# Jarvis73/PEMP

Measured on AMD Instinct MI355X. Metric: episodes/sec (PEMP stage-1 eval step, PASCAL-5i-shaped 1-shot, ResNet-50), higher is better.
Workload: dtype f32

## Files before the change

### pemp_amd/build.py

```python
import hashlib
import os
import subprocess
from concurrent.futures import ThreadPoolExecutor

HERE = os.path.dirname(os.path.abspath(__file__))
CSRC = os.path.join(HERE, "csrc")
OBJ = os.path.join(HERE, "_obj")
OUT = os.path.join(HERE, "libpemp_hip.so")
SOURCES = ("conv_igemm.hip", "conv_dma.hip", "conv_dma2.hip", "conv_panel.hip", "conv_row3.hip", "conv_stem_pool.hip", "conv_wgrad.hip", "train_ops.hip", "pool_misc.hip", "head.hip", "head_bwd.hip", "cedt.hip",
           "episode_io.hip", "dropout.hip", "cm_linear.hip", "pfenet.hip", "pfenet_bwd.hip", "canet.hip", "canet_bwd.hip", "rpmms.hip", "rpmms_bwd.hip")
FLAGS = ["-O3", "--offload-arch=gfx950", "-std=c++17", "-fPIC"]


def _headers():
    return [os.path.join(CSRC, f) for f in sorted(os.listdir(CSRC)) if f.endswith((".h", ".inc"))] + \
           [os.path.join(HERE, "..", "include", "pemp_hip.h")]


def csrc_digest():
    h = hashlib.sha1()
    for f in sorted(os.listdir(CSRC)):
        with open(os.path.join(CSRC, f), "rb") as fh:
            h.update(f.encode() + b"\0" + fh.read())
    with open(os.path.join(HERE, "..", "include", "pemp_hip.h"), "rb") as fh:
        h.update(fh.read())
    return h.hexdigest()[:12]


CONV_ENGINE = ("common.h", "conv_common.h", "conv_tiles.h", "conv_igemm.hip", "conv_dma.hip", "conv_dma2.hip", "conv_panel.hip", "conv_row3.hip", "conv_stem_pool.hip")


def conv_digest():
    h = hashlib.sha1()
    for f in CONV_ENGINE:
        with open(os.path.join(CSRC, f), "rb") as fh:
            h.update(f.encode() + b"\0" + fh.read())
    return h.hexdigest()[:12]


def needs_build():
    if not os.path.exists(OUT):
        return True
    t = os.path.getmtime(OUT)
    deps = [os.path.join(CSRC, f) for f in os.listdir(CSRC)] + [os.path.join(HERE, "..", "include", "pemp_hip.h")]
    return any(os.path.getmtime(d) > t for d in deps)


def _stamp(src, flags):
    h = hashlib.sha1(" ".join(flags).encode())
    for f in [src] + _headers():
        with open(f, "rb") as fh:
            h.update(fh.read())
# ... 41 lines not shown
```

### pemp_amd/csrc/conv_common.h

```cpp
#pragma once
#include "common.h"

namespace pemp {

typedef __attribute__((ext_vector_type(16))) float f32x16;
typedef __attribute__((ext_vector_type(4))) float v4f;
typedef __attribute__((ext_vector_type(8))) __bf16 bf16x8;
typedef __attribute__((ext_vector_type(2))) unsigned int u32x2;

#define PEMP_CONV_BF16_IO 0x100u

__device__ __forceinline__ v4f load_quad(const float* base, size_t off, unsigned bf16) {
    if (!bf16) return *(const v4f*)(base + off);
    const u32x2 r = *(const u32x2*)((const unsigned short*)base + off);
    return v4f{__builtin_bit_cast(float, r.x << 16), __builtin_bit_cast(float, r.x & 0xFFFF0000u),
               __builtin_bit_cast(float, r.y << 16), __builtin_bit_cast(float, r.y & 0xFFFF0000u)};
}

__device__ __forceinline__ unsigned int bf16_bits(float f) {
    const unsigned int u = __builtin_bit_cast(unsigned int, f);
    if ((u & 0x7FFFFFFFu) > 0x7F800000u) return (u >> 16) | 0x40u;
    return (u + 0x7FFFu + ((u >> 16) & 1u)) >> 16;
}

// ... 349 lines not shown

int launch_conv_dma(int shape, const ConvArgs& a, hipStream_t st);
bool conv_dma2_supported(const ConvArgs& a);
int launch_conv_dma2(int shape, const ConvArgs& a, hipStream_t st);
int launch_conv_dma2_group(int shape, ConvGroupArgs& g, hipStream_t st);
int launch_conv_dma2_hybrid(const ConvArgs& a, hipStream_t st);
int conv_dma2_hybrid_rows(int M, int Cout);
int launch_conv_dma2_bf16(int shape, const ConvArgs& a, hipStream_t st);
int launch_conv_dma2_db(int shape, ConvArgs a, void* ws, size_t ws_bytes, bool split, hipStream_t st);
struct SplitKPlan { int full, split, pieces; size_t ws_bytes; };
SplitKPlan conv_dma2_splitk_plan(int shape, const ConvArgs& a);
int launch_conv_dma2_splitk(int shape, ConvArgs a, void* ws, size_t ws_bytes, hipStream_t st);
int launch_conv_dma2_split3(int shape, ConvArgs a, void* ws, size_t ws_bytes, bool split, hipStream_t st);
int launch_conv_dma2_group_split3(int shape, ConvGroupArgs& g, hipStream_t st);
int launch_conv_dma2_split3_stats(int shape, const ConvArgs& a, hipStream_t st);
bool conv_dma2_split3_stats_shape(int shape);
int launch_conv_dma2_split3_persist(int shape, const ConvArgs& a, hipStream_t st);
bool conv_dma2_persist_out_split3(int shape);
int launch_conv_dma2_split3_pre(int shape, bool persistent, const ConvArgs& a, hipStream_t st);
bool conv_panel_supported(const ConvArgs& a);
int launch_conv_panel(int shape, const ConvArgs& a, hipStream_t st);
bool conv_row3_supported(const ConvArgs& a);
int launch_conv_row3(bool persistent, const ConvArgs& a, hipStream_t st);
int conv_dma2_simds();
int pack_split3(const float* w, void* out, int cout, int kpad, hipStream_t st);
int launch_conv_stem_pool(const ConvArgs& a, hipStream_t st);
int conv_stem_pool_out(int i);

template <class Kern> int allow_lds(Kern kern, size_t lds);
template <class Kern>
int persistent_grid(Kern kern, int threads, size_t lds, long long tiles, int& occ_cache, const char* what, int& grid_out) {
    if (!occ_cache) {
        const int rc = allow_lds(kern, lds);
        if (rc) return rc;
        int v = 0;
        hipError_t e = hipOccupancyMaxActiveBlocksPerMultiprocessor(&v, (const void*)kern, threads, lds);
        if (e != hipSuccess || v <= 0) {
            set_error("%s: occupancy query failed (%s, %d blocks)", what, hipGetErrorString(e), v);
            return -1;
        }
        occ_cache = v;
    }
    long long grid = (long long)occ_cache * (conv_dma2_simds() / 4);
    if (grid < 8) grid = 8;
    if (grid > tiles) grid = tiles;
    grid_out = (int)grid;
// ... 5 lines not shown
```

### pemp_amd/csrc/conv_igemm.hip

```cpp
#include "conv_tiles.h"

namespace pemp {


template <int BM, int BN, int WGM, bool STEM>
__global__ __launch_bounds__(256) void conv_igemm_kernel(ConvArgs a) {
    constexpr int WGN = 4 / WGM;
    constexpr int WM = BM / WGM, WN = BN / WGN;
    constexpr int TM = WM / 32, TN = WN / 32;
    constexpr int AL = BM / 32, BL = BN / 32;
    static_assert(TM >= 1 && TN >= 1, "wave tile");

    extern __shared__ __attribute__((aligned(16))) v4f smem[];
    v4f* As = smem;
    v4f* Bs = smem + 2 * 8 * BM;

    const int tid = threadIdx.x;
    const int lane = tid & 63;
    const int wave = tid >> 6;
    const int wm0 = (wave / WGN) * WM;
    const int wn0 = (wave % WGN) * WN;
    const int lr = lane & 31, lh = lane >> 5;

    const int ntn = a.Cout / BN;
// ... 255 lines not shown
    a.dil = d->dil; a.ldr = d->ldr; a.Kpad = d->Kpad; a.flags = d->flags;
    a.HoWo = d->Ho * d->Wo;
    a.M = d->N * a.HoWo;
    a.ntaps = ntaps;
    a.cin_steps = stem ? 1 : d->Cin / 32;
    a.nk = d->Kpad / 32;
    if (residual && !(d->flags & PEMP_CONV_OUT_SPLIT3_ALSO)) PEMP_REQUIRE(d->ldr >= d->Cout && d->ldr % 4 == 0 && ((uintptr_t)residual & 15) == 0, "conv2d: ldr must be >= Cout and x4, residual 16-byte aligned");
    a.sk_ws = nullptr; a.sk_cnt = nullptr; a.sk_full = 0; a.sk_S = 1;
    a.bm_first = 0;
    return 0;
}

static int conv2d_impl(const pemp_conv_desc* d, const float* x, const float* w, float* y, const float* scale, const float* shift,
                       const float* residual, const float* pad_value, void* ws, size_t ws_bytes, void* stream) {
    ConvArgs a;
    const int rc = conv_fill(d, x, w, y, scale, shift, residual, pad_value, a, false, true);
    if (rc) return rc;
    const bool stem = d->flags & PEMP_CONV_STEM4;
    int tile = d->tile;
    if (tile == 0) {
        tile = 3;
    }
    TileId t = decode_tile(tile);
    const bool out_split3 = d->flags & PEMP_CONV_OUT_SPLIT3;
    if (out_split3)
        PEMP_REQUIRE(t.family == TILE_SPLIT3 && !t.splitk && !t.panel && !ws && !stem && !residual && a.Cout % 32 == 0 && a.ldy == a.Cout,
                     "conv2d: PEMP_CONV_OUT_SPLIT3 needs an unsplit split3 tile id (41..44, 46, 47, 49, 146, 149), ldy == Cout, no residual / workspace");
    const bool also_split3 = d->flags & PEMP_CONV_OUT_SPLIT3_ALSO;
    if (also_split3) {
        PEMP_REQUIRE(t.presplit && !out_split3 && !ws && !stem && a.Cout % 32 == 0,
                     "conv2d: PEMP_CONV_OUT_SPLIT3_ALSO needs tile id 146 / 149, no PEMP_CONV_OUT_SPLIT3 / split-K / workspace / stem");
        PEMP_REQUIRE(residual && ((uintptr_t)residual & 15) == 0,
                     "conv2d: PEMP_CONV_OUT_SPLIT3_ALSO takes the pre-split tensor (16-byte aligned) in the residual argument; a residual is never read");
        const char *y0 = (const char*)y, *y1 = y0 + ((size_t)(a.M - 1) * a.ldy + a.Cout) * 4;
        const char *s0 = (const char*)residual, *s1 = s0 + (size_t)a.M * a.Cout * 6;
        PEMP_REQUIRE(y1 <= s0 || s1 <= y0, "conv2d: PEMP_CONV_OUT_SPLIT3_ALSO: y and the pre-split tensor overlap");
    }
    const bool res_s2 = d->flags & PEMP_CONV_RES_S2;
    PEMP_REQUIRE(res_s2 || !(d->flags & (PEMP_CONV_RES_HEVEN | PEMP_CONV_RES_WEVEN)), "conv2d: PEMP_CONV_RES_HEVEN / _WEVEN come with PEMP_CONV_RES_S2");
    if (res_s2) {
        PEMP_REQUIRE(residual && !out_split3 && !also_split3 && !(d->flags & PEMP_CONV_IN_SPLIT3) && !ws && !stem && !pad_value,
                     "conv2d: PEMP_CONV_RES_S2 needs a residual, no pre-split operands / PEMP_CONV_OUT_SPLIT3_ALSO / split-K / workspace / stem / padding value");
        PEMP_REQUIRE(t.family == TILE_SPLIT3 && t.exists && !t.splitk && !t.persistent && !t.presplit &&
                         (t.panel ? (a.nk == 2 || (a.nk == 4 && t.shape == 2)) : t.shape == 3),
                     "conv2d: PEMP_CONV_RES_S2 needs tile id 43, 72 with Kpad 64 or 128, or 71 with Kpad 64 (tile %d, Kpad %d: the persistent, split-K, "
                     "pre-split and fp32-chain ids have no strided-residual form)", tile, a.Kpad);
// ... 294 lines not shown
```

### pemp_amd/csrc/conv_tiles.h

```cpp
#pragma once
#include <initializer_list>
#include "conv_common.h"

namespace pemp {

struct TileShape { int bm, bn, wgm, nw, wgm3; };
inline constexpr TileShape kTileShapes[10] = {
    {0, 0, 0, 0, 0},
    {128, 128, 2, 4, 4},
    {128, 64, 2, 4, 4},
    {64, 64, 2, 4, 2},
    {128, 128, 4, 8, 4},
    {128, 64, 4, 8, 0},
    {256, 128, 4, 8, 8},
    {256, 256, 4, 8, 0},
    {32, 64, 2, 4, 0},
    {64, 64, 2, 4, 0},
};

template <int S, bool S3 = false>
struct Tile {
    static constexpr int BM = kTileShapes[S].bm, BN = kTileShapes[S].bn, NW = kTileShapes[S].nw;
    static constexpr int WGM = S3 ? kTileShapes[S].wgm3 : kTileShapes[S].wgm;
};
// ... 17 lines not shown
template <class Fam, int S = 1, class F>
int with_tile(int shape, F&& f) {
    if constexpr (S > 9) {
        set_error("conv: tile shape %d outside the kernel family", shape);
        return -1;
    } else {
        if constexpr ((Fam::shapes >> S) & 1u) {
            if (shape == S) return f(Tile<S, Fam::s3>{});
        }
        return with_tile<Fam, S + 1>(shape, f);
    }
}

enum TileFamily { TILE_NONE = 0, TILE_IGEMM, TILE_DMA, TILE_DMA2, TILE_SPLIT3 };
struct TileId {
    int family;
    int shape;
    bool splitk;
    bool persistent;
    bool exists;
    bool panel;
    bool presplit;
    bool row3;
};

inline TileId decode_tile(int id) {
    TileId t = {TILE_NONE, 0, false, false, false, false, false, false};
    const int decade = id / 10, s = id % 10;
    if (id == 146 || id == 149 || id == 246 || id == 249) {
        t.family = TILE_SPLIT3, t.shape = 6, t.exists = t.presplit = true, t.persistent = id % 10 == 9, t.row3 = id > 200;
        return t;
    }
    if (decade == 7 && in_family<FamPanel>(s)) {
        t.family = TILE_SPLIT3, t.shape = s, t.exists = t.panel = true;
        return t;
    }
    if (id < 1 || id > 56 || s == 0) return t;
    t.shape = s;
    if (decade == 0) t.family = TILE_IGEMM, t.exists = in_family<FamIgemm>(s);
    else if (decade == 1) t.family = TILE_DMA, t.exists = in_family<FamFp32>(s);
    else if (decade == 2) t.family = TILE_DMA2, t.exists = true;
    else if (decade == 3) t.family = TILE_DMA2, t.splitk = true, t.exists = in_family<FamSplitK>(s);
    else if (decade == 4 && (s == 7 || s == 9)) t.family = TILE_SPLIT3, t.persistent = t.exists = true, t.shape = s == 7 ? 3 : 6;
    else if (decade == 4) t.family = TILE_SPLIT3, t.exists = in_family<FamSplit3>(s);
    else t.family = TILE_SPLIT3, t.splitk = true, t.exists = in_family<FamSplit3>(s) && in_family<FamSplitK>(s);
    return t;
}

inline bool tile_cout_ok(int shape, int Cout) { return Cout % kTileShapes[shape].bn == 0; }
#define PEMP_REQUIRE_COUT(who, shape, Cout)                                                                              \
    do {                                                                                                                 \
// ... 39 lines not shown
```

### pemp_amd/ops.py

```python
import ctypes as C
import collections
import functools
import json
import os

import torch

from . import _lib
from ._lib import ConvDesc, CONV_RELU, CONV_SHIFT_PER_IMAGE, CONV_STEM4, CONV_POOL3S2, CONV_OUT_SPLIT3, CONV_IN_SPLIT3, CONV_OUT_SPLIT3_ALSO
from ._lib import CONV_RES_S2, CONV_RES_HEVEN, CONV_RES_WEVEN


def _stream():
    return C.c_void_p(torch.cuda.current_stream().cuda_stream)


def _p(t):
    return C.c_void_p(t.data_ptr()) if t is not None else C.c_void_p(0)


def _chk_dev(*ts):
    for t in ts:
        if t is not None and (not t.is_cuda):
            raise _lib.PempHipError("pemp_amd ops need device (cuda/HIP) tensors; there is no CPU path")
# ... 26 lines not shown
    def __init__(self, w, scale, shift, cin, cout, kh, kw, stride, pad, dil, kpad, stem, relu, w3=None, w3pool=None):
        self.w, self.scale, self.shift, self.w3, self.w3pool = w, scale, shift, w3, w3pool
        self.cin, self.cout, self.kh, self.kw = cin, cout, kh, kw
        self.stride, self.pad, self.dil, self.kpad, self.stem, self.relu = stride, pad, dil, kpad, stem, relu


_SHAPES = {1: (128, 128), 2: (128, 64), 3: (64, 64), 4: (128, 128), 5: (128, 64), 6: (256, 128), 7: (256, 256),
           8: (32, 64),
           9: (64, 64)}
Tile = collections.namedtuple("Tile", "shape family splitk persistent_of")
SPLIT3_PERSISTENT = {47: 43, 49: 46}
TILES = {base + s: Tile(_SHAPES[s], family, base in (30, 50), None)
         for family, base, shapes in (("igemm", 0, (1, 2, 3)),
                                      ("dma", 10, range(1, 8)),
                                      ("dma2", 20, range(1, 10)),
                                      ("dma2", 30, (1, 2, 4, 5, 6, 7)),
                                      ("split3", 40, (1, 2, 3, 4, 6)),
                                      ("split3", 50, (1, 2, 4, 6)))
         for s in shapes}
TILES.update({t: TILES[of]._replace(persistent_of=of) for t, of in SPLIT3_PERSISTENT.items()})
TILES.update({70 + s: Tile(_SHAPES[s], "split3", False, None) for s in (1, 2)})
TILES.update({146: Tile(_SHAPES[6], "split3", False, None), 149: Tile(_SHAPES[6], "split3", False, 146)})
TILES.update({246: Tile(_SHAPES[6], "split3", False, None), 249: Tile(_SHAPES[6], "split3", False, 246)})
_NO_TILE = Tile(None, None, False, None)


def tile_shape(t):
    return TILES.get(t, _NO_TILE).shape


TILE_VARIANTS = {t: TILES[t].shape for t in (13, 14, 12, 11, 15, 3, 17, 16, 23, 24, 22, 21, 25, 27, 26, 28, 29)}
SPLIT3_TILES = (43, 42, 41, 44, 46, 47, 49)
SPLIT3_SPLITK_TILES = (51, 52, 54, 56)
SPLIT3_DEFAULT_TILE = 43
SPLIT3_PANEL_TILES = (71, 72)
SPLIT3_PANEL = os.environ.get("PEMP_SPLIT3_PANEL", "1") != "0"
SPLIT3_PRESPLIT_TILES = (146, 149)
SPLIT3_PRESPLIT = os.environ.get("PEMP_SPLIT3_PRESPLIT", "1") != "0"
SPLIT3_ROW3_TILES = (246, 249)
SPLIT3_ROW3 = os.environ.get("PEMP_SPLIT3_ROW3", "1") != "0"
ROW3_STAGE_ROWS = 288
AUTOTUNE = True
PICK_HOOK = None
SPLITK = os.environ.get("PEMP_CONV_SPLITK", "1") != "0"
DEFAULT_TILE = 13
_TILE_CACHE = {}
_TILE_CACHE_FILE = os.environ.get("PEMP_TILE_CACHE")
WGRAD_PICKS = {}
if _TILE_CACHE_FILE and os.path.exists(_TILE_CACHE_FILE):
    with open(_TILE_CACHE_FILE) as _f:
        for _k, _v in json.load(_f).items():
            _key = json.loads(_k)
            if _key and _key[0] == "wgrad":
                WGRAD_PICKS[tuple(_key[1:])] = tuple(_v) if isinstance(_v, list) else int(_v)
            else:
                _TILE_CACHE[tuple(_key)] = int(_v)


def save_picks():
    if not _TILE_CACHE_FILE:
        return
    out = {json.dumps([int(v) for v in k]): t for k, t in _TILE_CACHE.items()}
    out.update({json.dumps(["wgrad"] + [int(v) for v in k]): (list(t) if isinstance(t, tuple) else t) for k, t in WGRAD_PICKS.items()})
    with open(_TILE_CACHE_FILE, "w") as f:
# ... 100 lines not shown
            and pad_value is None and not splitk and not per_image_shift and n * h * w * ldx * 4 < lim
            and n * ho * wo * max(ldy, ldr) * 4 < lim)


SPLIT3_RES_S2_TILES = (43, 72, 71)


def res_s2_tiles(p):
    if p.w3 is None or p.stem:
        return ()
    panel = p.kh == 1 and p.kw == 1 and p.pad == 0
    return tuple(t for t in SPLIT3_RES_S2_TILES
                 if t == 43 or (panel and p.cout % _tile_bn(t) == 0 and (p.kpad == 64 or (p.kpad == 128 and t == 72))))


def row3_stage_rows(w, dil):
    return 256 + 2 * dil + dil * ((255 + 2 * dil + w - 1) // w)


def _row3_ok(p, w, residual, pad_value, out_split3, also_split3, per_image_shift):
    return (SPLIT3_ROW3 and (p.kh, p.kw, p.stride) == (3, 3, 1) and p.pad == p.dil and residual is None
            and pad_value is None and not out_split3 and also_split3 is None and not per_image_shift
            and row3_stage_rows(w, p.dil) <= ROW3_STAGE_ROWS)


def pack_split3(w):
    co, kpad = w.shape
    if w.dtype != torch.float32 or not w.is_contiguous() or kpad % 32:
        raise ValueError("pack_split3: a contiguous fp32 [Cout, Kpad] with Kpad % 32 == 0")
    out = torch.empty((co, kpad // 32, 3, 32), dtype=torch.bfloat16, device=w.device)
    _lib.check(_lib.load().pemp_pack_split3_bf16(_p(w), _p(out), co, kpad, _stream()), "pemp_pack_split3_bf16")
    return out


def hybrid_rows(n, ho, wo, cout):
    d = ConvDesc(n, ho, wo, 32, 32, ho, wo, cout, cout, 1, 1, 1, 0, 1, 0, 32, 0, 29)
    return int(_lib.load().pemp_conv2d_hybrid_rows(C.byref(d)))


def pack_conv_weight(w_oihw, stem4=False):
    co, ci, kh, kw = w_oihw.shape
    w = w_oihw.detach().permute(0, 2, 3, 1).contiguous().float()
    if stem4:
        if ci > 4:
            raise ValueError("stem4 packing needs Cin <= 4")
        k = kh * kw * 4
# ... 44 lines not shown
        raise ValueError(f"{who}: out shape {tuple(out.shape)} != {(n, ho, wo, p.cout)}")
    ldr = 0
    if residual is not None:
        ldr = _nhwc(residual, "residual", dtype)
        if residual_stride == 2:
            rn, hr, wr, rc = residual.shape
            if (rn, rc) != (n, p.cout) or (hr - 1) // 2 + 1 != ho or (wr - 1) // 2 + 1 != wo:
                raise ValueError(f"{who}: a stride-2 residual of shape {tuple(residual.shape)} does not cover the output {tuple(out.shape)}")
        elif tuple(residual.shape) != tuple(out.shape):
            raise ValueError(f"{who}: residual shape mismatch")
    elif residual_stride != 1:
        raise ValueError(f"{who}: residual_stride without a residual")
    return n, h, w, cin, ldx, ho, wo, out, ldy, ldr


def conv2d(x, p, out=None, residual=None, shift_override=None, per_image_shift=False, relu=None, tile=0,
           pad_value=None, splitk=False, dropblock=None, out_split3=False, x_split3=False, also_split3=None, residual_stride=1):
    if out_split3 or x_split3:
        what = "a pre-split output" if out_split3 else "a pre-split input"
        if p.w3 is None or p.stem:
            raise ValueError(f"conv2d: {what} needs a split3 layer (ConvParams.w3), not the fp32 chain or a stem")
        if splitk or dropblock is not None:
            raise ValueError(f"conv2d: {what} has no split-K / DropBlock form")
        if out_split3 and tile and (tile not in SPLIT3_TILES + SPLIT3_PRESPLIT_TILES):
            raise ValueError(f"conv2d: a pre-split output needs an unsplit split3 tile id, got {tile}")
        if x_split3 and (p.kh * p.kw == 1 or per_image_shift or p.cin % 32 or p.cout % 128):
            raise ValueError("conv2d: a pre-split input needs a multi-tap conv with Cin % 32 == 0 and Cout % 128 == 0, no per-image shift")
    if also_split3 is not None and (not x_split3 or out_split3 or residual is not None):
        raise ValueError("conv2d: a second, pre-split output needs a pre-split input (x_split3), no out_split3, no residual")
    if (tile in SPLIT3_PRESPLIT_TILES + SPLIT3_ROW3_TILES) != bool(x_split3) and (tile or not x_split3):
        raise ValueError(f"conv2d: the tile ids {SPLIT3_PRESPLIT_TILES + SPLIT3_ROW3_TILES} and x_split3 come together (tile {tile})")
    res_s2 = residual_stride == 2
    if residual_stride not in (1, 2):
        raise ValueError(f"conv2d: residual_stride must be 1 or 2, got {residual_stride}")
    if res_s2:
        if p.w3 is None or p.stem or x.dtype != torch.float32:
            raise ValueError("conv2d: a stride-2 residual needs a split3 layer (ConvParams.w3) on fp32 activations")
        if residual is None or out_split3 or x_split3 or also_split3 is not None or pad_value is not None or splitk or dropblock is not None:
            raise ValueError("conv2d: a stride-2 residual comes with a residual and without pre-split operands, padding value, split-K or DropBlock")
        if tile and tile not in res_s2_tiles(p):
            raise ValueError(f"conv2d: a stride-2 residual needs one of the tile ids {res_s2_tiles(p)} for this layer, got {tile}")
    if x.dtype == torch.bfloat16 and not x_split3:
        return _conv2d_bf16(x, p, out, residual, shift_override, per_image_shift, relu, tile, pad_value)
    n, h, w, cin, ldx, ho, wo, out, ldy, ldr = _conv_geom("conv2d", x, p, out, residual, x_split3=x_split3, out_split3=out_split3,
                                                          residual_stride=residual_stride)
    if also_split3 is not None and _split3_dims(also_split3, "also_split3") != (n, ho, wo, p.cout):
        raise ValueError(f"conv2d: also_split3 shape {tuple(also_split3.shape)} != {split3_shape(n, ho, wo, p.cout)}")
# ... 54 lines not shown
            ws, ws_bytes = _splitk_ws(lib, d, x.device)
            _check_sk(lib, lib.pemp_conv2d_padv_splitk_nhwc_f32(C.byref(d), _p(x), _p(pw), _p(out), _p(p.scale), _p(shift), _p(residual),
                                                                _p(pad_value), C.c_void_p(ws), ws_bytes, _stream()), ws,
                      "pemp_conv2d_padv_splitk_nhwc_f32")
        elif sk:
            ws, ws_bytes = _splitk_ws(lib, d, x.device)
            _check_sk(lib, lib.pemp_conv2d_splitk_nhwc_f32(C.byref(d), _p(x), _p(pw), _p(out), _p(p.scale), _p(shift), _p(residual),
                                                           C.c_void_p(ws), ws_bytes, _stream()), ws, "pemp_conv2d_splitk_nhwc_f32")
        elif pad_value is None:
            _lib.check(lib.pemp_conv2d_nhwc_f32(C.byref(d), _p(x), _p(pw), _p(out), _p(p.scale), _p(shift),
                                                _p(residual), _stream()), "pemp_conv2d_nhwc_f32")
        else:
            _lib.check(lib.pemp_conv2d_padv_nhwc_f32(C.byref(d), _p(x), _p(pw), _p(out), _p(p.scale), _p(shift),
                                                     _p(residual), _p(pad_value), _stream()), "pemp_conv2d_padv_nhwc_f32")

    if tile == 0:
        key = (p.cin, p.cout, p.kh, p.kw, p.stride, p.pad, p.dil, (6 if dropblock is not None else 4) if splitk else int(p.stem) + (7 if dropblock is not None else 0),
               n, h, w, int(residual is not None and also_split3 is None), int(pad_value is not None)) + ((3,) if s3 else ())
        if x_split3 or out_split3:
            key += (146,) * int(x_split3) + (17,) * int(out_split3) + (64,) * int(also_split3 is not None)
            row3 = bool(x_split3) and _row3_ok(p, w, residual, pad_value, out_split3, also_split3, per_image_shift)
            if row3:
                key += (246,)
            cands = lambda: _fits(list(SPLIT3_PRESPLIT_TILES if x_split3 else SPLIT3_TILES) +
                                  (list(SPLIT3_ROW3_TILES) if row3 and PICK_HOOK is None else []), p.cout)
        elif res_s2:
            panel = _panel_ok(p, n, ho, wo, ldx, ldy, ldr, h, w, pad_value, splitk, per_image_shift) \
                and residual.numel() // p.cout * ldr * 4 < 1 << 31
            key += (128,) + ((71,) if panel else ())
            cands = lambda: _fits([t for t in res_s2_tiles(p) if panel or t not in SPLIT3_PANEL_TILES], p.cout)
        elif s3:
            panel = _panel_ok(p, n, ho, wo, ldx, ldy, ldr, h, w, pad_value, splitk, per_image_shift)
            if panel:
                key += (71,)
            cands = lambda: _fits(list(SPLIT3_TILES) + (list(SPLIT3_SPLITK_TILES) if splitk else []) +
                                  (list(SPLIT3_PANEL_TILES) if panel else []), p.cout)
        else:
            def cands():
                ids = list(GROUP_TILES if dropblock is not None else TILE_VARIANTS) + (list(SPLITK_TILES) if splitk else [])
                if 29 in ids and not (hybrid_rows(n, ho, wo, p.cout) and dma2_supported(x, p)):
                    ids.remove(29)
                return _fits(ids, p.cout)
        tile = _choose_tile(key, n * ho * wo, launch, cands,
                            SPLIT3_PRESPLIT_TILES[0] if x_split3 else SPLIT3_DEFAULT_TILE if s3 else DEFAULT_TILE + (10 if dropblock is not None else 0))
    launch(tile)
    return out


def stem_pool_supported(p):
    return (p.stem and p.w3pool is not None and (p.kh, p.kw, p.stride, p.pad, p.dil) == (7, 7, 2, 3, 1) and p.kpad == 224
            and p.cout % 64 == 0)


def stem_pool(x, p, out=None):
    lib = _lib.load()
    if not stem_pool_supported(p):
        raise ValueError("stem_pool: a 7x7 / stride 2 / pad 3 NHWC4 stem with split weights (ConvParams.w3pool)")
    _chk_dev(x, p.w3pool, out)
    ldx = _nhwc(x, "x")
# ... 1091 lines not shown
```

### scratch/conv_trace_layers.py

```python
import collections
import csv
import sys

trace, per_step = sys.argv[1], int(sys.argv[2])
steps = int(sys.argv[3]) if len(sys.argv) > 3 else 20
rows = sorted(csv.DictReader(open(trace)), key=lambda r: int(r["Start_Timestamp"]))
conv = [r for r in rows if any(k in r["Kernel_Name"] for k in ("conv_dma", "conv_igemm", "conv_stem_pool", "conv_panel", "conv_row3"))][-steps * per_step:]
dur = lambda r: (int(r["End_Timestamp"]) - int(r["Start_Timestamp"])) / 1e3
pos = collections.defaultdict(list)
for i, r in enumerate(conv):
    pos[i % per_step].append(r)
print(f"conv launches per step {per_step}, steps {steps}: conv {sum(map(dur, conv)) / steps / 1e3:.3f} ms per step")
print(f"{'pos':>3} {'mean us':>9} {'grid':>8} {'wg':>4}  kernel")
for p in range(per_step):
    rs = pos[p]
    r = rs[-1]
    name = r["Kernel_Name"].split("(")[0].replace("void pemp::", "").replace("pemp::", "")
    g = r.get("Grid_Size", r.get("Grid_Size_X", "")); wg = r.get("Workgroup_Size", r.get("Workgroup_Size_X", ""))
    print(f"{p:>3} {sum(map(dur, rs)) / len(rs):9.1f} {g:>8} {wg:>4}  {name}")
```

### scratch/s3_layers_bench.py

```python
import argparse
import hashlib
import os
import sys

import torch

sys.path.insert(0, os.path.dirname(os.path.dirname(os.path.abspath(__file__))))
from pemp_amd import ops

UNSPLIT = (43, 42, 41, 44, 46, 47, 49)
SPLIT = (52, 51, 54, 56)
PANEL = ops.SPLIT3_PANEL_TILES
PRESPLIT = ops.SPLIT3_PRESPLIT_TILES
ROW3 = ops.SPLIT3_ROW3_TILES
LAYERS = ((256, 1024, 1, 1, True, False), (512, 1024, 1, 1, False, False), (1024, 256, 1, 1, False, False),
          (256, 256, 3, 2, False, False), (128, 512, 1, 1, True, False), (1024, 512, 1, 1, False, False),
          (256, 256, 3, 2, False, True),
          (64, 256, 1, 1, True, False, 1, 101), (64, 256, 1, 1, False, False, 1, 101), (256, 512, 1, 1, False, False, 2, 101),
          (128, 128, 3, 1, False, False), (128, 128, 3, 1, False, False, 2, 101), (64, 64, 3, 1, False, False, 1, 101),
          (512, 128, 1, 1, False, False),
          (64, 256, 1, 1, True, False, 1, 51, 101),
          (64, 64, 3, 1, False, False, 2, 101),
          (256, 256, 3, 12, False, True))


def timed(fn, reps, n=5):
    for _ in range(2):
        fn()
    e0, e1 = torch.cuda.Event(enable_timing=True), torch.cuda.Event(enable_timing=True)
    best, worst = 1e9, 0.0
    for _ in range(reps):
        e0.record()
        for _ in range(n):
            fn()
        e1.record()
        e1.synchronize()
        us = e0.elapsed_time(e1) / n * 1e3
        best, worst = min(best, us), max(worst, us)
    return best, worst


def presplit(x):
    h = x.to(torch.bfloat16)
# ... 15 lines not shown
    packed = packed.contiguous()
    prm = ops.ConvParams(packed, None, torch.randn(cout, generator=g).to(dev), cin, cout, 1, 1, 1, 0, 1, kpad, False, True, ops.pack_split3(packed))
    res = torch.randn(N, HR, HR, cout, generator=g).to(dev)
    ref = ops.conv2d(x, prm, residual=res[:, ::2, ::2, :].contiguous(), tile=43).clone()
    out = torch.empty_like(ref)
    fl = 2.0 * N * HW * HW * cout * cin
    cells = []
    for tile in keep(ops.res_s2_tiles(prm)):
        run = lambda: ops.conv2d(x, prm, residual=res, residual_stride=2, out=out, tile=tile)
        out.zero_()
        run()
        same = torch.equal(out, ref)
        us, worst = timed(run, reps)
        cells.append(f"{tile}: {us:7.1f}..{worst:6.1f}us {fl / us / 1e6:5.1f}TF{'' if same else ' !'}")
    print(f"{name:>16} k1 d1 res1 | " + " | ".join(cells), flush=True)
    print(f"{'':>16} hash 43={digest(ref)}", flush=True)


def main():
    ap = argparse.ArgumentParser()
    ap.add_argument("--only", default="", help="cin-cout-kK[-padv]: one layer")
    ap.add_argument("--reps", type=int, default=3)
    ap.add_argument("--ids", default="", help="comma-separated tile ids: only these are timed (a counter run of one kernel)")
    ap.add_argument("--res", type=int, choices=(0, 1), default=None, help="run the selected layers without / with a residual, whatever their row says")
    args = ap.parse_args()
    dev = torch.device("cuda:0")
    N = 50
    keep = lambda ids: tuple(t for t in ids if not args.ids or str(t) in args.ids.split(","))
    for layer in LAYERS:
        cin, cout, k, dil, has_res, padv = layer[:6]
        stride, HW = layer[6:8] if len(layer) > 6 else (1, 51)
        RS2 = layer[8] if len(layer) > 8 else 0
        has_res = has_res if args.res is None or RS2 else bool(args.res)
        M = N * HW * HW
        HO = (HW - 1) // stride + 1
        name = f"{cin}-{cout}-k{k}" + (f"-d{dil}" if k == 3 and dil > 2 else "") + ("-padv" if padv else "") + (f"-s{stride}" if stride > 1 else "") + (f"-hw{HW}-res{int(has_res)}" if HW != 51 else "") + ("-rs2" if RS2 else "")
        if args.only and name not in args.only.split(","):
            continue
        if RS2:
            rs2_row(dev, N, HW, RS2, cin, cout, name, keep, args.reps)
            continue
        g = torch.Generator().manual_seed(cin * 7 + cout * 3 + k)
        buf = torch.empty(M + 4, cin, device=dev)
        buf[:M] = torch.randn(M, cin, generator=g).to(dev)
        buf[M:] = torch.randn(cin, generator=g).to(dev)
        x, pv = buf[:M].view(N, HW, HW, cin), buf[M]
        w = (torch.randn(cout, cin, k, k, generator=g) * (1.0 / (cin * k * k) ** 0.5)).to(dev)
        packed, kpad = ops.pack_conv_weight(w)
        packed = packed.contiguous()
        prm = ops.ConvParams(packed, None, torch.randn(cout, generator=g).to(dev), cin, cout, k, k, stride, dil if k == 3 else 0, dil, kpad,
                             False, True, ops.pack_split3(packed))
        res = torch.randn(N, HO, HO, cout, generator=g).to(dev) if has_res else None
        pad_value = pv if padv else None
        out = torch.empty(N, HO, HO, cout, device=dev)
        fl = 2.0 * N * HO * HO * cout * k * k * cin
        ref = ops.conv2d(x, prm, residual=res, pad_value=pad_value, tile=43).clone()
        cells, hashes = [], [f"43={digest(ref)}"]
        panel = PANEL if k == 1 and kpad <= 256 and not padv else ()
        for tile in keep(UNSPLIT + panel + SPLIT):
            if cout % ops._tile_bn(tile):
                continue
            run = lambda: ops.conv2d(x, prm, residual=res, pad_value=pad_value, out=out, tile=tile)
            run()
            same = torch.equal(out, ref)
            if tile in SPLIT:
                hashes.append(f"{tile}=" + ("43" if same else digest(out)))
            us, worst = timed(run, args.reps)
            mark = "" if same else (" ~" if tile in SPLIT else " !")
            cells.append(f"{tile}: {us:7.1f}..{worst:6.1f}us {fl / us / 1e6:5.1f}TF{mark}")
            if tile not in SPLIT and not same:
                hashes.append(f"{tile}=MISMATCH:{digest(out)}")
        if k > 1 and cout % 128 == 0:
            sbuf = torch.zeros((M + 4) * cin * 3, dtype=torch.bfloat16, device=dev)
            sbuf[:(M + 1) * cin * 3] = presplit(buf[:M + 1]).reshape(-1)
            xs, pvs = sbuf[:M * cin * 3].view(N, HW, HW, cin // 32, 3, 32), sbuf[M * cin * 3:(M + 1) * cin * 3].view(cin // 32, 3, 32)
            row3 = ROW3 if k == 3 and stride == 1 and not has_res and not padv and ops.row3_stage_rows(HW, dil) <= ops.ROW3_STAGE_ROWS else ()
            for tile in keep(PRESPLIT + row3):
                run = lambda: ops.conv2d(xs, prm, residual=res, pad_value=pvs if padv else None, out=out, tile=tile, x_split3=True)
                out.zero_()
                run()
                same = torch.equal(out, ref)
                us, worst = timed(run, args.reps)
                cells.append(f"{tile}: {us:7.1f}..{worst:6.1f}us {fl / us / 1e6:5.1f}TF{'' if same else ' !'}")
            if not has_res:
                want = presplit(ref)
                outs = torch.empty_like(want)
                for tile in keep(PRESPLIT):
                    run = lambda: ops.conv2d(xs, prm, pad_value=pvs if padv else None, out=out, tile=tile, x_split3=True, also_split3=outs)
                    out.zero_()
                    run()
                    same = torch.equal(out, ref) and torch.equal(outs.view(torch.int16), want.view(torch.int16))
                    us, worst = timed(run, args.reps)
                    cells.append(f"{tile}+s: {us:7.1f}..{worst:6.1f}us{'' if same else ' !'}")
                del want, outs
            del sbuf, xs, pvs
        if k == 1 and not has_res:
            want = presplit(ref)
            outs = torch.empty_like(want)
            for tile in keep((43, 42, 41, 44, 46, 47, 49) if not args.ids else ()):
                if cout % ops._tile_bn(tile):
                    continue
                run = lambda: ops.conv2d(x, prm, out=outs, tile=tile, out_split3=True)
                run()
                same = torch.equal(outs.view(torch.int16), want.view(torch.int16))
                us, worst = timed(run, args.reps)
                cells.append(f"{tile}s: {us:7.1f}..{worst:6.1f}us{'' if same else ' !'}")
            del want, outs
        print(f"{name:>16} k{k} d{dil} res{int(has_res)} | " + " | ".join(cells), flush=True)
        print(f"{'':>16} hash " + " ".join(hashes), flush=True)
    print("(146 / 149 / 246 / 249: on the pre-split input; NNs: id NN writing a pre-split output, ! = not the split of id 43's;")
    print(" NNN+s: id NNN writing fp32 and the pre-split copy, ! = either differs)")
    print("(! = an unsplit id differs from id 43; ~ = a split-K id differs from id 43, expected where it splits)")


if __name__ == "__main__":
    main()
```

Measured before the change: 1552.

## Add persistent triple-buffered ring conv kernel for 1x1 split3 layers

Adds a new persistent 1x1 convolution kernel (tile 349) using a three-stage A ring and two-stage B buffer filled by direct buffer-to-LDS loads. Scheduling barriers interleave MFMA, LDS reads and DMA issues, and the next tile's prefetch overlaps the current tile's epilogue. It is added as an autotune candidate for eligible 1x1 split3 layers, aiming to hide global memory latency behind the bf16 split3 MFMA chain. It uses 144 KB of LDS per block, which limits occupancy, and adds autotune and code complexity.

```diff
diff --git a/pemp_amd/build.py b/pemp_amd/build.py
--- a/pemp_amd/build.py
+++ b/pemp_amd/build.py
@@ -7,7 +7,7 @@
 CSRC = os.path.join(HERE, "csrc")
 OBJ = os.path.join(HERE, "_obj")
 OUT = os.path.join(HERE, "libpemp_hip.so")
-SOURCES = ("conv_igemm.hip", "conv_dma.hip", "conv_dma2.hip", "conv_panel.hip", "conv_row3.hip", "conv_stem_pool.hip", "conv_wgrad.hip", "train_ops.hip", "pool_misc.hip", "head.hip", "head_bwd.hip", "cedt.hip",
+SOURCES = ("conv_igemm.hip", "conv_dma.hip", "conv_dma2.hip", "conv_panel.hip", "conv_row3.hip", "conv_ring.hip", "conv_stem_pool.hip", "conv_wgrad.hip", "train_ops.hip", "pool_misc.hip", "head.hip", "head_bwd.hip", "cedt.hip",
            "episode_io.hip", "dropout.hip", "cm_linear.hip", "pfenet.hip", "pfenet_bwd.hip", "canet.hip", "canet_bwd.hip", "rpmms.hip", "rpmms_bwd.hip")
 FLAGS = ["-O3", "--offload-arch=gfx950", "-std=c++17", "-fPIC"]
 
@@ -27,7 +27,7 @@
     return h.hexdigest()[:12]
 
 
-CONV_ENGINE = ("common.h", "conv_common.h", "conv_tiles.h", "conv_igemm.hip", "conv_dma.hip", "conv_dma2.hip", "conv_panel.hip", "conv_row3.hip", "conv_stem_pool.hip")
+CONV_ENGINE = ("common.h", "conv_common.h", "conv_tiles.h", "conv_igemm.hip", "conv_dma.hip", "conv_dma2.hip", "conv_panel.hip", "conv_row3.hip", "conv_ring.hip", "conv_stem_pool.hip")
 
 
 def conv_digest():
diff --git a/pemp_amd/csrc/conv_common.h b/pemp_amd/csrc/conv_common.h
--- a/pemp_amd/csrc/conv_common.h
+++ b/pemp_amd/csrc/conv_common.h
@@ -395,6 +395,8 @@
 int launch_conv_panel(int shape, const ConvArgs& a, hipStream_t st);
 bool conv_row3_supported(const ConvArgs& a);
 int launch_conv_row3(bool persistent, const ConvArgs& a, hipStream_t st);
+bool conv_ring_supported(const ConvArgs& a);
+int launch_conv_ring(const ConvArgs& a, hipStream_t st);
 int conv_dma2_simds();
 int pack_split3(const float* w, void* out, int cout, int kpad, hipStream_t st);
 int launch_conv_stem_pool(const ConvArgs& a, hipStream_t st);
diff --git a/pemp_amd/csrc/conv_igemm.hip b/pemp_amd/csrc/conv_igemm.hip
--- a/pemp_amd/csrc/conv_igemm.hip
+++ b/pemp_amd/csrc/conv_igemm.hip
@@ -301,6 +301,13 @@
         tile = 3;
     }
     TileId t = decode_tile(tile);
+    if (t.ring) {
+        PEMP_REQUIRE(!ws && !pad_value && conv_ring_supported(a),
+                     "conv2d: tile %d unsupported: needs a 1x1 conv without padding on fp32 activations with Kpad == Cin >= 128 and Cout %% 128 == 0, the "
+                     "fp32 output or PEMP_CONV_OUT_SPLIT3 (ldy == Cout); no residual, PEMP_CONV_OUT_SPLIT3_ALSO, PEMP_CONV_IN_SPLIT3, PEMP_CONV_RES_S2, "
+                     "padding value, stem, split-K or workspace; operands < 2 GiB", tile);
+        return launch_conv_ring(a, (hipStream_t)stream);
+    }
     const bool out_split3 = d->flags & PEMP_CONV_OUT_SPLIT3;
     if (out_split3)
         PEMP_REQUIRE(t.family == TILE_SPLIT3 && !t.splitk && !t.panel && !ws && !stem && !residual && a.Cout % 32 == 0 && a.ldy == a.Cout,
diff --git a/pemp_amd/csrc/conv_ring.hip b/pemp_amd/csrc/conv_ring.hip
--- /dev/null
+++ b/pemp_amd/csrc/conv_ring.hip
@@ -0,0 +1,302 @@
+#include "conv_tiles.h"
+
+namespace pemp {
+
+typedef __attribute__((address_space(3))) void* lptr_t;
+
+constexpr int RING_BM = 256, RING_BN = 128, RING_NW = 8;
+constexpr int RING_AQ = RING_BM * 8, RING_BQ = RING_BN * 12;
+constexpr int RING_AL = RING_AQ / (RING_NW * 64), RING_BL = RING_BQ / (RING_NW * 64);
+static_assert(RING_AQ % (RING_NW * 64) == 0 && RING_BQ % (RING_NW * 64) == 0, "whole DMA rounds");
+constexpr size_t ring_lds() { return (size_t)(3 * RING_AQ + 2 * RING_BQ) * sizeof(v4f); }
+static_assert(ring_lds() == 147456 && ring_lds() <= 160 * 1024, "LDS of a CU");
+constexpr int RING_MIN_NK = 4;
+
+enum RingWait { RING_STEP, RING_FIRST };
+constexpr int ring_behind(RingWait w, int stores = 0) { return w == RING_STEP ? RING_AL : RING_AL + stores + RING_BL + RING_AL; }
+
+template <int OUT>
+__global__ __launch_bounds__(RING_NW * 64) __attribute__((amdgpu_waves_per_eu(2))) void conv_ring_kernel(ConvArgs a) {
+#if defined(__HIP_DEVICE_COMPILE__)
+    constexpr int BM = RING_BM, BN = RING_BN, NW = RING_NW;
+    constexpr int WM = BM / NW, TN = BN / 32;
+    static_assert(WM == 32, "one 32-row strip per wave");
+    constexpr int AL = RING_AL, BL = RING_BL, AQ = RING_AQ, BQ = RING_BQ;
+    constexpr int NMF = 6 * TN, NDS = 2 + 3 * TN;
+    static_assert(NDS + BL + AL <= NMF, "one LDS read / one DMA per MFMA slot");
+    constexpr int NST = TN * (OUT == 0 ? 4 : 6);
+    static_assert(ring_behind(RING_FIRST, NST) <= 63, "vmcnt range");
+    static_assert(NW * 256 <= AQ, "one 4 KB transpose patch per wave inside ONE A stage");
+
+    extern __shared__ __attribute__((aligned(16))) v4f smem[];
+    v4f* As = smem;
+    v4f* Bs = smem + 3 * AQ;
+
+    const int tid = threadIdx.x;
+    const int lane = tid & 63;
+    const int wave = __builtin_amdgcn_readfirstlane(tid >> 6);
+    const int wm0 = wave * WM;
+    const int lr = lane & 31, lh = lane >> 5;
+
+    const int ntn = a.Cout / BN;
+    const XcdTileRange tr((a.M + BM - 1) / BM * ntn, (int)blockIdx.x, (int)gridDim.x);
+    if (tr.idx >= tr.count) return;
+    int j = tr.idx;
+    int m0 = ((tr.first + j) / ntn) * BM, n0 = ((tr.first + j) % ntn) * BN;
+
+    const int p = tid & 7;
+    const int r = tid >> 3;
+    const int sq = p ^ ((r >> 1) & 7);
+    const __amdgpu_buffer_rsrc_t rx = __builtin_amdgcn_make_buffer_rsrc((void*)a.x, 0, 0x80000000u, 0x00020000);
+    const __amdgpu_buffer_rsrc_t rw = __builtin_amdgcn_make_buffer_rsrc((void*)a.w, 0, 0x80000000u, 0x00020000);
+
+    unsigned a_voff[AL], b_voff[BL];
+    auto a_offsets = [&](const int m0_, const bool ok_) {
+#pragma unroll
+        for (int i = 0; i < AL; ++i) {
+            const int m = m0_ + r + NW * 8 * i;
+            const bool in = ok_ && m < a.M;
+            const int mm = in ? m : 0;
+            const int img = mm / a.HoWo;
+            const int rem = mm - img * a.HoWo;
+            const int ho = rem / a.Wo;
+            const int wo = rem - ho * a.Wo;
+            a_voff[i] = in ? (unsigned)(((img * a.H + ho * a.stride) * a.W + wo * a.stride) * a.ldx + sq * 4) * 4u : 0x80000000u;
+        }
+    };
+    auto b_offsets = [&](const int n0_, const bool ok_) {
+#pragma unroll
+        for (int i = 0; i < BL; ++i) {
+            const int q = i * NW * 64 + tid, row = q / 12, pos = q - row * 12;
+            const int src = PEMP_SPLIT3_SWZ(row, pos);
+            b_voff[i] = ok_ ? (unsigned)((n0_ + row) * a.Kpad * 6 + src * 16) : 0x80000000u;
+        }
+    };
+    a_offsets(m0, true);
+    b_offsets(n0, true);
+    const int nk = a.nk;
+
+#define PEMP_RING_DMA_A(ao_, k_)                                                                                  \
+    do {                                                                                                          \
+        const int so_ = __builtin_amdgcn_readfirstlane((k_) * 128);                                               \
+        _Pragma("unroll") for (int i = 0; i < AL; ++i)                                                            \
+            __builtin_amdgcn_raw_ptr_buffer_load_lds(rx, (lptr_t)(As + (ao_) + i * NW * 64 + wave * 64), 16, a_voff[i], so_, 0, 0); \
+    } while (0)
+#define PEMP_RING_DMA_B(bo_, k_)                                                                                  \
+    do {                                                                                                          \
+        const int so_ = __builtin_amdgcn_readfirstlane((k_) * 192);                                               \
+        _Pragma("unroll") for (int i = 0; i < BL; ++i)                                                            \
+            __builtin_amdgcn_raw_ptr_buffer_load_lds(rw, (lptr_t)(Bs + (bo_) + i * NW * 64 + wave * 64), 16, b_voff[i], so_, 0, 0); \
+    } while (0)
+
+    const int rsw = (lr >> 1) & 7;
+    const int arow = (wm0 + lr) * 8;
+    const int brow3 = lr * 12, bsw3 = (lr >> 2) & 3;
+    v4f af3[2][2], bf3[2][TN][3];
+#define PEMP_RING_READ(dst_, ao_, bo_, j_)                                                                        \
+    do {                                                                                                          \
+        const v4f* Ab_ = As + (ao_);                                                                              \
+        const v4f* Bb_ = Bs + (bo_);                                                                              \
+        const int p0_ = (4 * (j_) + 2 * lh) ^ rsw, p1_ = (4 * (j_) + 2 * lh + 1) ^ rsw;                           \
+        const int pb_ = (2 * (j_) + lh) ^ bsw3;                                                                   \
+        af3[dst_][0] = Ab_[arow + p0_];                                                                           \
+        af3[dst_][1] = Ab_[arow + p1_];                                                                           \
+        _Pragma("unroll") for (int ni = 0; ni < TN; ++ni)                                                         \
+            _Pragma("unroll") for (int pl = 0; pl < 3; ++pl)                                                      \
+                bf3[dst_][ni][pl] = Bb_[brow3 + ni * 32 * 12 + pl * 4 + pb_];                                     \
+    } while (0)
+
+#define PEMP_RING_MMA(src_)                                                                                       \
+    do {                                                                                                          \
+        bf16x8 ah_, am_, al_;                                                                                     \
+        split3_bf16(af3[src_][0], af3[src_][1], ah_, am_, al_);                                                   \
+        _Pragma("unroll") for (int ni = 0; ni < TN; ++ni) {                                                       \
+            const bf16x8 bh_ = __builtin_bit_cast(bf16x8, bf3[src_][ni][0]);                                      \
+            const bf16x8 bm_ = __builtin_bit_cast(bf16x8, bf3[src_][ni][1]);                                      \
+            const bf16x8 bl_ = __builtin_bit_cast(bf16x8, bf3[src_][ni][2]);                                      \
+            acc[ni] = __builtin_amdgcn_mfma_f32_32x32x16_bf16(al_, bh_, acc[ni], 0, 0, 0);                        \
+            acc[ni] = __builtin_amdgcn_mfma_f32_32x32x16_bf16(ah_, bl_, acc[ni], 0, 0, 0);                        \
+            acc[ni] = __builtin_amdgcn_mfma_f32_32x32x16_bf16(am_, bm_, acc[ni], 0, 0, 0);                        \
+            acc[ni] = __builtin_amdgcn_mfma_f32_32x32x16_bf16(am_, bh_, acc[ni], 0, 0, 0);                        \
+            acc[ni] = __builtin_amdgcn_mfma_f32_32x32x16_bf16(ah_, bm_, acc[ni], 0, 0, 0);                        \
+            acc[ni] = __builtin_amdgcn_mfma_f32_32x32x16_bf16(ah_, bh_, acc[ni], 0, 0, 0);                        \
+        }                                                                                                         \
+    } while (0)
+
+#define PEMP_RING_STEP(TAIL_)                                                                                     \
+    do {                                                                                                          \
+        PEMP_RING_READ(1, ao, bo, 1);                                                                             \
+        __builtin_amdgcn_sched_barrier(0);                                                                        \
+        PEMP_RING_MMA(0);                                                                                         \
+        __builtin_amdgcn_sched_barrier(0);                                                                        \
+         \
+        __builtin_amdgcn_s_waitcnt(0xC07F);              \
+        if (TAIL_) asm volatile("s_waitcnt vmcnt(%0) lgkmcnt(0)" ::"n"(ring_behind(RING_STEP)) : "memory");       \
+        else asm volatile("s_waitcnt lgkmcnt(0)" ::: "memory");                                                   \
+        __builtin_amdgcn_s_barrier();                                                        \
+        __builtin_amdgcn_sched_barrier(0);                                                                        \
+        if (TAIL_) {                                                                                              \
+            PEMP_RING_DMA_B(bo, kb);                                                                              \
+            PEMP_RING_DMA_A(ao, ka);                                                                              \
+            PEMP_RING_READ(0, an, bn, 0);                                                                         \
+        }                                                                                                         \
+        PEMP_RING_MMA(1);                \
+        if (TAIL_) {                     \
+            _Pragma("unroll") for (int k_ = 0; k_ < NMF; ++k_) {                                                  \
+                __builtin_amdgcn_sched_group_barrier(0x008, 1, 0);                                                \
+                if (k_ < BL + AL) __builtin_amdgcn_sched_group_barrier(0x020, 1, 0);                              \
+                else if (k_ < BL + AL + NDS) __builtin_amdgcn_sched_group_barrier(0x100, 1, 0);                   \
+            }                                                                                                     \
+        }                                                                                                         \
+        __builtin_amdgcn_sched_barrier(0);                                                                        \
+        {                                                                                  \
+            const int t_ = ao;                                                                                    \
+            ao = an;                                                                                              \
+            an = ann;                                                                                             \
+            ann = t_;                                                                                             \
+            const int u_ = bo;                                                                                    \
+            bo = bn;                                                                                              \
+            bn = u_;                                                                                              \
+        }                                                                                                         \
+    } while (0)
+
+    int ao = 0, an = AQ, ann = 2 * AQ, bo = 0, bn = BQ;
+    PEMP_RING_DMA_A(ao, 0);
+    PEMP_RING_DMA_B(bo, 0);
+    PEMP_RING_DMA_A(an, 1);
+    PEMP_RING_DMA_B(bn, 1);
+    PEMP_RING_DMA_A(ann, 2);
+    {
+        constexpr int V0 = ring_behind(RING_FIRST);
+        __builtin_amdgcn_s_waitcnt((V0 & 15) | 0x0F70 | ((V0 >> 4) << 14));
+        asm volatile("s_waitcnt vmcnt(%0)" ::"n"(V0) : "memory");
+    }
+    __builtin_amdgcn_s_barrier();
+    __builtin_amdgcn_sched_barrier(0);
+
+    const int c4_ = (lane & 7) * 4;
+    for (;;) {
+        f32x16 acc[TN];
+#pragma unroll
+        for (int ni = 0; ni < TN; ++ni)
+#pragma unroll
+            for (int e = 0; e < 16; ++e) acc[ni][e] = 0.f;
+        const int jn = j + tr.step;
+        const bool more = jn < tr.count;
+        const int m0n = more ? ((tr.first + jn) / ntn) * BM : m0, n0n = more ? ((tr.first + jn) % ntn) * BN : n0;
+
+        v4f scv[OUT == 0 ? TN : 1], shv[OUT == 0 ? TN : 1], sc8[OUT == 0 ? 1 : TN][2], sh8[OUT == 0 ? 1 : TN][2];
+        const bool per_img = a.flags & PEMP_CONV_SHIFT_PER_IMAGE;
+        auto epi_loads = [&]() {
+            if constexpr (OUT == 0) {
+#pragma unroll
+                for (int ni = 0; ni < TN; ++ni) {
+                    const int n = n0 + ni * 32 + c4_;
+                    scv[ni] = a.scale ? *(const v4f*)(a.scale + n) : v4f{1.f, 1.f, 1.f, 1.f};
+                    shv[ni] = (a.shift && !per_img) ? *(const v4f*)(a.shift + n) : v4f{0.f, 0.f, 0.f, 0.f};
+                }
+            } else {
+#pragma unroll
+                for (int ni = 0; ni < TN; ++ni) conv_split3_affine(a, n0 + ni * 32 + (lane & 3) * 8, sc8[ni], sh8[ni]);
+            }
+        };
+
+        PEMP_RING_READ(0, ao, bo, 0);
+        int ka = 3, kb = 2;
+        for (int kt = 0; kt + 3 < nk; ++kt) {
+            PEMP_RING_STEP(true);
+            ++ka;
+            ++kb;
+        }
+        a_offsets(m0n, more);
+        ka = 0;
+        PEMP_RING_STEP(true);
+        b_offsets(n0n, more);
+        ka = 1;
+        kb = 0;
+        PEMP_RING_STEP(true);
+        const int al_ = ao, bl_ = bo;
+        PEMP_RING_STEP(false);
+        epi_loads();
+
+        __builtin_amdgcn_s_waitcnt(0x0F70);
+        asm volatile("s_waitcnt vmcnt(0)" ::: "memory");
+        float* patch = (float*)(As + al_ + wave * 256);
+        if constexpr (OUT == 0) {
+#pragma unroll
+            for (int ni = 0; ni < TN; ++ni) {
+                PEMP_CONV_PATCH_PUT(patch, acc[ni], lr, lh);
+                asm volatile("s_waitcnt lgkmcnt(0)" ::: "memory");
+                conv_patch_store_f32(a, patch, m0 + wm0, n0 + ni * 32, lane, scv[ni], shv[ni], per_img, nullptr, 0u);
+                asm volatile("s_waitcnt lgkmcnt(0)" ::: "memory");
+            }
+        } else {
+#pragma unroll
+            for (int ni = 0; ni < TN; ++ni) {
+                PEMP_CONV_PATCH_PUT(patch, acc[ni], lr, lh);
+                asm volatile("s_waitcnt lgkmcnt(0)" ::: "memory");
+                conv_store_split3_to(a, (unsigned short*)a.y, patch, m0 + wm0, n0 + ni * 32, lane, sc8[ni], sh8[ni]);
+                asm volatile("s_waitcnt lgkmcnt(0)" ::: "memory");
+            }
+        }
+        if (!more) {
+            asm volatile("s_waitcnt vmcnt(0)" ::: "memory");
+            break;
+        }
+
+        __builtin_amdgcn_s_barrier();
+        PEMP_RING_DMA_B(bl_, 1);
+        PEMP_RING_DMA_A(al_, 2);
+        constexpr int VF = ring_behind(RING_FIRST, NST), VP = ring_behind(RING_FIRST);
+        if (m0 + wm0 + WM <= a.M) {
+            __builtin_amdgcn_s_waitcnt((VF & 15) | 0x0F70 | ((VF >> 4) << 14));
+            asm volatile("s_waitcnt vmcnt(%0)" ::"n"(VF) : "memory");
+        } else {
+            __builtin_amdgcn_s_waitcnt((VP & 15) | 0x0F70 | ((VP >> 4) << 14));
+            asm volatile("s_waitcnt vmcnt(%0)" ::"n"(VP) : "memory");
+        }
+        __builtin_amdgcn_s_barrier();
+        __builtin_amdgcn_sched_barrier(0);
+        j = jn;
+        m0 = m0n;
+        n0 = n0n;
+    }
+#endif
+}
+#undef PEMP_RING_STEP
+#undef PEMP_RING_MMA
+#undef PEMP_RING_READ
+#undef PEMP_RING_DMA_B
+#undef PEMP_RING_DMA_A
+
+bool conv_ring_supported(const ConvArgs& a) {
+    if (a.flags & (PEMP_CONV_IN_SPLIT3 | PEMP_CONV_OUT_SPLIT3_ALSO | PEMP_CONV_RES_S2 | PEMP_CONV_RES_HEVEN | PEMP_CONV_RES_WEVEN | PEMP_CONV_STEM4 |
+                   PEMP_CONV_POOL3S2 | PEMP_CONV_BF16_IO))
+        return false;
+    if (a.res || a.padv || a.stats || a.rowmask || a.sk_S > 1 || a.sk_ws || a.bm_first) return false;
+    if (a.KH != 1 || a.KW != 1 || a.pad != 0 || a.stride < 1) return false;
+    if (a.Cin % 32 || a.Kpad != a.Cin || a.nk != a.Kpad / 32 || a.nk < RING_MIN_NK || a.ldx < a.Cin || a.Cout % RING_BN) return false;
+    if ((a.flags & PEMP_CONV_OUT_SPLIT3) && a.ldy != a.Cout) return false;
+    return conv_dma2_supported(a) && (long long)a.Cout * a.Kpad * 6 < (1ll << 31);
+}
+
+int launch_conv_ring(const ConvArgs& a, hipStream_t st) {
+    if (!conv_ring_supported(a)) {
+        set_error("conv split3 ring: unsupported (needs a 1x1 conv without padding on fp32 activations, Kpad == Cin >= %d, Cout %% 128 == 0, "
+                  "the fp32 or PEMP_CONV_OUT_SPLIT3 output without residual / second output / padding value / workspace)", 32 * RING_MIN_NK);
+        return -1;
+    }
+    const int tiles = cdiv(a.M, RING_BM) * (a.Cout / RING_BN);
+    static int occ[2] = {0, 0};
+    int grid = 0;
+    if (a.flags & PEMP_CONV_OUT_SPLIT3) {
+        const int rc = persistent_grid(conv_ring_kernel<1>, RING_NW * 64, ring_lds(), tiles, occ[1], "conv split3 ring", grid);
+        if (rc) return rc;
+        return launch_with_lds(conv_ring_kernel<1>, grid, RING_NW * 64, ring_lds(), st, a, "conv_ring/out_split3");
+    }
+    const int rc = persistent_grid(conv_ring_kernel<0>, RING_NW * 64, ring_lds(), tiles, occ[0], "conv split3 ring", grid);
+    if (rc) return rc;
+    return launch_with_lds(conv_ring_kernel<0>, grid, RING_NW * 64, ring_lds(), st, a, "conv_ring");
+}
+
+}
diff --git a/pemp_amd/csrc/conv_tiles.h b/pemp_amd/csrc/conv_tiles.h
--- a/pemp_amd/csrc/conv_tiles.h
+++ b/pemp_amd/csrc/conv_tiles.h
@@ -63,11 +63,16 @@
     bool panel;
     bool presplit;
     bool row3;
+    bool ring;
 };
 
 inline TileId decode_tile(int id) {
-    TileId t = {TILE_NONE, 0, false, false, false, false, false, false};
+    TileId t = {TILE_NONE, 0, false, false, false, false, false, false, false};
     const int decade = id / 10, s = id % 10;
+    if (id == 349) {
+        t.family = TILE_SPLIT3, t.shape = 6, t.exists = t.persistent = t.ring = true;
+        return t;
+    }
     if (id == 146 || id == 149 || id == 246 || id == 249) {
         t.family = TILE_SPLIT3, t.shape = 6, t.exists = t.presplit = true, t.persistent = id % 10 == 9, t.row3 = id > 200;
         return t;
diff --git a/pemp_amd/ops.py b/pemp_amd/ops.py
--- a/pemp_amd/ops.py
+++ b/pemp_amd/ops.py
@@ -72,6 +72,7 @@
 TILES.update({70 + s: Tile(_SHAPES[s], "split3", False, None) for s in (1, 2)})
 TILES.update({146: Tile(_SHAPES[6], "split3", False, None), 149: Tile(_SHAPES[6], "split3", False, 146)})
 TILES.update({246: Tile(_SHAPES[6], "split3", False, None), 249: Tile(_SHAPES[6], "split3", False, 246)})
+TILES.update({349: Tile(_SHAPES[6], "split3", False, 46)})
 _NO_TILE = Tile(None, None, False, None)
 
 
@@ -90,6 +91,9 @@
 SPLIT3_ROW3_TILES = (246, 249)
 SPLIT3_ROW3 = os.environ.get("PEMP_SPLIT3_ROW3", "1") != "0"
 ROW3_STAGE_ROWS = 288
+SPLIT3_RING_TILES = (349,)
+SPLIT3_RING = os.environ.get("PEMP_SPLIT3_RING", "1") != "0"
+RING_MIN_K = 128
 AUTOTUNE = True
 PICK_HOOK = None
 SPLITK = os.environ.get("PEMP_CONV_SPLITK", "1") != "0"
@@ -236,6 +240,12 @@
     return (SPLIT3_ROW3 and (p.kh, p.kw, p.stride) == (3, 3, 1) and p.pad == p.dil and residual is None
             and pad_value is None and not out_split3 and also_split3 is None and not per_image_shift
             and row3_stage_rows(w, p.dil) <= ROW3_STAGE_ROWS)
+
+
+def _ring_ok(p, x_split3, residual, pad_value, also_split3, splitk, res_s2=False):
+    return (SPLIT3_RING and PICK_HOOK is None and p.w3 is not None and not p.stem and (p.kh, p.kw, p.pad) == (1, 1, 0)
+            and p.cin % 32 == 0 and p.kpad == p.cin and p.kpad >= RING_MIN_K and p.cout % 128 == 0 and not x_split3 and residual is None
+            and pad_value is None and also_split3 is None and not splitk and not res_s2 and p.cout * p.kpad * 6 < 1 << 31)
 
 
 def pack_split3(w):
@@ -326,7 +336,7 @@
             raise ValueError(f"conv2d: {what} needs a split3 layer (ConvParams.w3), not the fp32 chain or a stem")
         if splitk or dropblock is not None:
             raise ValueError(f"conv2d: {what} has no split-K / DropBlock form")
-        if out_split3 and tile and (tile not in SPLIT3_TILES + SPLIT3_PRESPLIT_TILES):
+        if out_split3 and tile and (tile not in SPLIT3_TILES + SPLIT3_PRESPLIT_TILES + SPLIT3_RING_TILES):
             raise ValueError(f"conv2d: a pre-split output needs an unsplit split3 tile id, got {tile}")
         if x_split3 and (p.kh * p.kw == 1 or per_image_shift or p.cin % 32 or p.cout % 128):
             raise ValueError("conv2d: a pre-split input needs a multi-tap conv with Cin % 32 == 0 and Cout % 128 == 0, no per-image shift")
@@ -427,8 +437,12 @@
             row3 = bool(x_split3) and _row3_ok(p, w, residual, pad_value, out_split3, also_split3, per_image_shift)
             if row3:
                 key += (246,)
+            ring = _ring_ok(p, x_split3, residual, pad_value, also_split3, splitk)
+            if ring:
+                key += (349,)
             cands = lambda: _fits(list(SPLIT3_PRESPLIT_TILES if x_split3 else SPLIT3_TILES) +
-                                  (list(SPLIT3_ROW3_TILES) if row3 and PICK_HOOK is None else []), p.cout)
+                                  (list(SPLIT3_ROW3_TILES) if row3 and PICK_HOOK is None else []) +
+                                  (list(SPLIT3_RING_TILES) if ring else []), p.cout)
         elif res_s2:
             panel = _panel_ok(p, n, ho, wo, ldx, ldy, ldr, h, w, pad_value, splitk, per_image_shift) \
                 and residual.numel() // p.cout * ldr * 4 < 1 << 31
@@ -436,10 +450,13 @@
             cands = lambda: _fits([t for t in res_s2_tiles(p) if panel or t not in SPLIT3_PANEL_TILES], p.cout)
         elif s3:
             panel = _panel_ok(p, n, ho, wo, ldx, ldy, ldr, h, w, pad_value, splitk, per_image_shift)
+            ring = _ring_ok(p, x_split3, residual, pad_value, also_split3, splitk)
+            if ring:
+                key += (349,)
             if panel:
                 key += (71,)
             cands = lambda: _fits(list(SPLIT3_TILES) + (list(SPLIT3_SPLITK_TILES) if splitk else []) +
-                                  (list(SPLIT3_PANEL_TILES) if panel else []), p.cout)
+                                  (list(SPLIT3_RING_TILES) if ring else []) + (list(SPLIT3_PANEL_TILES) if panel else []), p.cout)
         else:
             def cands():
                 ids = list(GROUP_TILES if dropblock is not None else TILE_VARIANTS) + (list(SPLITK_TILES) if splitk else [])
diff --git a/scratch/conv_trace_layers.py b/scratch/conv_trace_layers.py
--- a/scratch/conv_trace_layers.py
+++ b/scratch/conv_trace_layers.py
@@ -5,7 +5,7 @@
 trace, per_step = sys.argv[1], int(sys.argv[2])
 steps = int(sys.argv[3]) if len(sys.argv) > 3 else 20
 rows = sorted(csv.DictReader(open(trace)), key=lambda r: int(r["Start_Timestamp"]))
-conv = [r for r in rows if any(k in r["Kernel_Name"] for k in ("conv_dma", "conv_igemm", "conv_stem_pool", "conv_panel", "conv_row3"))][-steps * per_step:]
+conv = [r for r in rows if any(k in r["Kernel_Name"] for k in ("conv_dma", "conv_igemm", "conv_stem_pool", "conv_panel", "conv_row3", "conv_ring"))][-steps * per_step:]
 dur = lambda r: (int(r["End_Timestamp"]) - int(r["Start_Timestamp"])) / 1e3
 pos = collections.defaultdict(list)
 for i, r in enumerate(conv):
diff --git a/scratch/s3_layers_bench.py b/scratch/s3_layers_bench.py
--- a/scratch/s3_layers_bench.py
+++ b/scratch/s3_layers_bench.py
@@ -12,6 +12,7 @@
 SPLIT = (52, 51, 54, 56)
 PANEL = ops.SPLIT3_PANEL_TILES
 PRESPLIT = ops.SPLIT3_PRESPLIT_TILES
+RING = getattr(ops, "SPLIT3_RING_TILES", ())
 ROW3 = ops.SPLIT3_ROW3_TILES
 LAYERS = ((256, 1024, 1, 1, True, False), (512, 1024, 1, 1, False, False), (1024, 256, 1, 1, False, False),
           (256, 256, 3, 2, False, False), (128, 512, 1, 1, True, False), (1024, 512, 1, 1, False, False),
@@ -19,6 +20,7 @@
           (64, 256, 1, 1, True, False, 1, 101), (64, 256, 1, 1, False, False, 1, 101), (256, 512, 1, 1, False, False, 2, 101),
           (128, 128, 3, 1, False, False), (128, 128, 3, 1, False, False, 2, 101), (64, 64, 3, 1, False, False, 1, 101),
           (512, 128, 1, 1, False, False),
+          (512, 256, 1, 1, False, False), (256, 256, 1, 1, False, False),
           (64, 256, 1, 1, True, False, 1, 51, 101),
           (64, 64, 3, 1, False, False, 2, 101),
           (256, 256, 3, 12, False, True))
@@ -80,6 +82,7 @@
     ap.add_argument("--only", default="", help="cin-cout-kK[-padv]: one layer")
     ap.add_argument("--reps", type=int, default=3)
     ap.add_argument("--ids", default="", help="comma-separated tile ids: only these are timed (a counter run of one kernel)")
+    ap.add_argument("--producers", action="store_true", help="with --ids: time the selected ids as producers of a pre-split output too")
     ap.add_argument("--res", type=int, choices=(0, 1), default=None, help="run the selected layers without / with a residual, whatever their row says")
     args = ap.parse_args()
     dev = torch.device("cuda:0")
@@ -115,7 +118,8 @@
         ref = ops.conv2d(x, prm, residual=res, pad_value=pad_value, tile=43).clone()
         cells, hashes = [], [f"43={digest(ref)}"]
         panel = PANEL if k == 1 and kpad <= 256 and not padv else ()
-        for tile in keep(UNSPLIT + panel + SPLIT):
+        ring = RING if k == 1 and kpad >= 128 and not has_res and not padv and cout % 128 == 0 else ()
+        for tile in keep(UNSPLIT + ring + panel + SPLIT):
             if cout % ops._tile_bn(tile):
                 continue
             run = lambda: ops.conv2d(x, prm, residual=res, pad_value=pad_value, out=out, tile=tile)
@@ -155,7 +159,7 @@
         if k == 1 and not has_res:
             want = presplit(ref)
             outs = torch.empty_like(want)
-            for tile in keep((43, 42, 41, 44, 46, 47, 49) if not args.ids else ()):
+            for tile in keep((43, 42, 41, 44, 46, 47, 49) + ring if not args.ids or args.producers else ()):
                 if cout % ops._tile_bn(tile):
                     continue
                 run = lambda: ops.conv2d(x, prm, out=outs, tile=tile, out_split3=True)
```

Result: faster. 1577, median of 6 (+1.6%).
